# martende/findex

Measured on AMD Instinct MI355X. Metric: rank_queries_per_sec, higher is better.
Workload: dtype u64

## Files before the change

### findex_amd/csrc/fmx_search4.h

```cpp
#pragma once
#include <type_traits>
#include "fmx_device.h"

namespace fmx {

constexpr int kSThreads = 256;

__device__ __forceinline__ uint32_t fetch4(const uint8_t *__restrict__ pat, uint64_t pos) {
  if (pos >= 4) {
    uint32_t d;
    __builtin_memcpy(&d, pat + pos - 4, 4);
    return __builtin_bswap32(d);
  }
  uint32_t r = 0;
  for (uint32_t j = 0; j < (uint32_t)pos; j++) r |= (uint32_t)pat[pos - 1 - j] << (8 * j);
  return r;
}


__device__ __forceinline__ uint32_t pat_chunk(const uint8_t *__restrict__ pat, const uint64_t *__restrict__ own,
                                              uint64_t end, uint32_t len, uint32_t j) {
  const uint32_t have = len > 4u * j ? len - 4u * j : 0u;
  const uint64_t pos = end - 4ull * j;
  const uint32_t back = have >= 4u ? 4u : have;
  const uint8_t *src = have ? pat + (pos - back) : reinterpret_cast<const uint8_t *>(own);
  uint32_t d;
  __builtin_memcpy(&d, src, 4);
  return __builtin_bswap32(d) >> (8u * (4u - (back ? back : 4u)));
}

#ifndef FMX_SEARCH_WAVES
#define FMX_SEARCH_WAVES 6
#endif
#ifdef FMX_SEARCHLOG
static __device__ unsigned long long g_searchlog[1u << 15][4];
#endif
#ifndef FMX_SEARCH_WAVES_G2
#define FMX_SEARCH_WAVES_G2 5
#endif
template <bool WIDE, uint32_t LAYOUT, uint32_t KT, uint32_t JT, uint32_t RW, bool R3T, bool G2 = false, bool KX = false>
__global__ __launch_bounds__(kSThreads) __attribute__((amdgpu_waves_per_eu(G2 ? FMX_SEARCH_WAVES_G2 : FMX_SEARCH_WAVES, 8))) void k_search4(DevIndex ix, const uint4 *__restrict__ ktab, const uint8_t *__restrict__ kdense,
                                                        uint32_t ksigma, const uint4 *__restrict__ kext, const uint4 *__restrict__ kovf,
                                                        const uint4 *__restrict__ jtab, const uint32_t jc,
                                                        const unsigned long long *__restrict__ r3tab, const uint8_t *__restrict__ pat,
                                                        const PatOff po,
                                                        uint64_t *__restrict__ sp_out, uint64_t *__restrict__ ep_out,
                                                        uint32_t k, unsigned long long *__restrict__ counters, const uint64_t pk_cap,
                                                        const uint32_t spin) {
  static_assert(!G2 || LAYOUT == kLayoutOneHot, "pairs of lanes serve the one-hot layout only");
  static_assert(!KX || (KT != 0 && JT == 2u && RW == 0u && LAYOUT == kLayoutOneHot), "level KT + 1 serves the kernels with pairs of row jump entries");
  constexpr int G = G2 ? 2 : Lay<LAYOUT>::G;
  constexpr uint32_t P = 64 / G;
  constexpr uint32_t RG = G2 ? 4u : (uint32_t)G;
  constexpr uint32_t R = LAYOUT == kLayoutBytes ? 2u : 1u;
#ifdef FMX_SEARCHLOG
  const unsigned long long sl_t0 = __builtin_amdgcn_s_memrealtime();
  unsigned long long sl_t1 = 0;
  uint32_t sl_batches = 0;
#endif
  if (threadIdx.x == 0 && blockIdx.x < kCensusBlocks) {
    counters[(size_t)kCounterSlots * kCounterStride + 2u * blockIdx.x] = __builtin_amdgcn_s_memrealtime();
    if (blockIdx.x == 0) counters[(size_t)kCounterSlots * kCounterStride + 2u * kCensusBlocks] = gridDim.x;
  }
  if (spin & 0xFFFFu) {
    const unsigned long long c0 = __builtin_amdgcn_s_memrealtime();
    while (__builtin_amdgcn_s_memrealtime() - c0 < (spin & 0xFFFFu)) __builtin_amdgcn_s_sleep(32);
  }
  __shared__ uint4 s_tab[256];
  __shared__ uint8_t s_dense[KT ? 256 : 4];
  __shared__ uint16_t s_slot[KT ? 256 : 4];
  for (int c = threadIdx.x; c < 256; c += blockDim.x) {
    if (KT) { s_dense[c] = kdense[c]; s_slot[c] = ix.slot[c]; }
    const uint64_t cf = ix.cf[c];
    const uint16_t s = ix.slot[c];
    uint64_t vb = 0;
    if (s < kSlotEof) vb = LAYOUT == kLayoutBytes ? (uint64_t)s + 2 : (uint64_t)(uintptr_t)ix.bv + (uint64_t)s * ix.nblocks * kBlockBytes;
    else if (s == kSlotEof) vb = 1;
    s_tab[c] = make_uint4((uint32_t)cf, (uint32_t)(cf >> 32), (uint32_t)vb, (uint32_t)(vb >> 32));
  }
  __syncthreads();
  const LaneConst lc = lane_const<G2 ? 4 : G>();
  const uint32_t t = G2 ? (threadIdx.x & 1u) : lc.t;
  const uint32_t lane_off = t * 16;
  uint32_t steps = 0, reqs = 0;
  struct Blk { uint4 a, b; };
  auto blk_load = [&](uint64_t vb, uint32_t b1, uint32_t upto) -> Blk {
    const uint64_t at = vb + lane_off + (uint64_t)b1 * kBlockBytes;
    Blk w;
    w.a = load_line16(at);
    w.b = make_uint4(0, 0, 0, 0);
    if constexpr (G2) {
      if (upto >= 192u) w.b = load_line16(at + 32);
    }
    return w;
  };
  auto blk_rank = [&](const Blk &w, uint32_t m1) -> uint64_t {
    if constexpr (G2) return rank_finish_g2<WIDE>(Blk2{w.a, w.b}, m1, t);
    else return rank_finish<WIDE>(w.a, m1, lc);
  };
  auto blk_bit = [&](const Blk &w, uint32_t m1) -> uint32_t {
    if constexpr (G2) return payload_bit_g2(Blk2{w.a, w.b}, m1, t);
    else return payload_bit(w.a, m1, lc);
  };
  constexpr uint32_t RB = 1u;
  auto gbc0 = [&](uint32_t v) -> uint32_t { if constexpr (G2) return pair_bcast<0>(v); else return group_bcast<G, 0>(v); };
  auto gbc1 = [&](uint32_t v) -> uint32_t { if constexpr (G2) return pair_bcast<1>(v); else return group_bcast<G, 1>(v); };
  const uint32_t wave = (blockIdx.x * kSThreads + threadIdx.x) >> 6;
  const uint32_t nwaves = gridDim.x * (kSThreads / 64);
  const uint32_t grp = (threadIdx.x & 63) / G;
  const uint32_t nbatch = (k + P - 1) / P;
  constexpr bool kPool = G2 || RW != 0u;
  const uint32_t tix_area = kPool ? (spin >> 16) & 0xFFu : 0u;
  const bool miss_none = JT != 0u && (spin >> 31) != 0u;
  uint32_t nstatic = nbatch;
  if (tix_area) {
    const uint32_t rounds = nbatch / nwaves, held = (spin >> 24) & 0xFu;
    if (rounds >= held + 2u) nstatic = (rounds - held) * nwaves;
  }
  constexpr bool kStage = LAYOUT != kLayoutBytes;
  constexpr uint32_t kStageBytes = G2 ? 2048 : 1024, kStagePad = 16;
  __shared__ __attribute__((aligned(16))) uint32_t s_pat[kSThreads / 64][2][kStage ? (kStagePad + kStageBytes + 16) / 4 : 4];
  uint32_t par = 0;
  constexpr bool kFold = (JT && RW == 0u) || RW != 0u;
  constexpr uint32_t kParkCap = RW ? 128u : (G2 ? 96u : 64u);
  __shared__ uint64_t s_park_row[kFold ? kSThreads / 64 : 1][kFold ? kParkCap : 1];
  __shared__ uint32_t s_park_pid[kFold ? kSThreads / 64 : 1][kFold ? kParkCap : 1];
  __shared__ uint32_t s_park_it[kFold ? kSThreads / 64 : 1][kFold ? kParkCap : 1];
  uint32_t npark = 0;
  constexpr uint32_t kRowsCap = 64u + P;
  __shared__ uint64_t s_rows_row[RW ? kSThreads / 64 : 1][RW ? kRowsCap : 1];
  __shared__ uint64_t s_rows_end[RW ? kSThreads / 64 : 1][RW ? kRowsCap : 1];
  __shared__ uint32_t s_rows_pid[RW ? kSThreads / 64 : 1][RW ? kRowsCap : 1];
  __shared__ uint32_t s_rows_it[RW ? kSThreads / 64 : 1][RW ? kRowsCap : 1];
  __shared__ uint32_t s_rows_len[RW ? kSThreads / 64 : 1][RW ? kRowsCap : 1];
  uint32_t nrows = 0;
  uint32_t rsteps = 0, rlooks = 0;
  auto emit = [&](uint32_t q, uint64_t a, uint64_t b) {
    if (pk_cap != ~0ull) {
      unsigned long long *pk = reinterpret_cast<unsigned long long *>(sp_out);
      const uint64_t w = b - a;
      if (w >= kPackWide) {
        const unsigned long long slot = atomicAdd(pk + k, 1ull);
        if (slot < pk_cap) { pk[(uint64_t)k + 1 + 2 * slot] = q; pk[(uint64_t)k + 2 + 2 * slot] = b; }
      }
      pk[q] = a | ((w < kPackWide ? w : kPackWide) << 40);
    } else {
      sp_out[q] = a;
      ep_out[q] = b;
    }
  };
  const uint32_t wave_in_wg = (uint32_t)__builtin_amdgcn_readfirstlane((int)(threadIdx.x >> 6));
  const uint32_t lane64 = threadIdx.x & 63u;
  const uint64_t pat_addr = (uint64_t)(uintptr_t)pat;
  auto load_off_raw = [&](uint64_t bt, uint64_t &v0, uint64_t &v1) {
    const uint64_t pid = bt * P + grp;
    const uint64_t *p = po.at(pid < k ? pid : (uint64_t)k - 1);
    v0 = p[0];
    v1 = p[1];
  };
  auto fix_off = [&](uint64_t bt, uint64_t v0, uint64_t v1, uint64_t &e, uint32_t &len) {
    const uint64_t pid = bt * P + grp;
    const uint64_t q = pid < k ? pid : (uint64_t)k - 1;
    const uint64_t b = po.fixed ? q * po.fixed : v0;
    e = po.fixed ? (q + 1) * po.fixed : v1;
    len = pid < k ? (uint32_t)(e - b) : 0u;
  };
  struct Stage { uint4 w; uint4 w2; uint64_t base; bool ok; };
  auto stage_issue = [&](uint64_t e, uint32_t len) {
    const uint64_t b = e - len;
    const uint64_t b0 = ((uint64_t)__builtin_amdgcn_readfirstlane((int)(uint32_t)(b >> 32)) << 32) | (uint32_t)__builtin_amdgcn_readfirstlane((int)(uint32_t)b);
    const uint64_t e1 = ((uint64_t)(uint32_t)__builtin_amdgcn_readlane((int)(uint32_t)(e >> 32), 63) << 32) | (uint32_t)__builtin_amdgcn_readlane((int)(uint32_t)e, 63);
    Stage st;
    const uint64_t al = (pat_addr + b0) & ~15ull;
    const uint64_t span = pat_addr + e1 - al;
    st.ok = kStage && span <= kStageBytes;
    st.base = al - pat_addr;
    st.w = make_uint4(0, 0, 0, 0);
    if (st.ok && 16ull * lane64 < span) st.w = load_line16(al + 16u * lane64);
    st.w2 = make_uint4(0, 0, 0, 0);
    if constexpr (G2) {
      if (st.ok && 1024ull + 16ull * lane64 < span) st.w2 = load_line16(al + 1024u + 16u * lane64);
    }
    return st;
  };
  auto stage_park = [&](const Stage &st, uint32_t area) {
    if (st.ok) *reinterpret_cast<uint4 *>(s_pat[wave_in_wg][area] + (kStagePad + 16u * lane64) / 4) = st.w;
    if constexpr (G2) {
      if (st.ok) *reinterpret_cast<uint4 *>(s_pat[wave_in_wg][area] + (kStagePad + 1024u + 16u * lane64) / 4) = st.w2;
    }
  };
  constexpr uint32_t NT = KT ? KT / 4 : 1;
  struct Tail { uint32_t c[NT]; };
  uint64_t end0, end1, raw2a, raw2b;
  uint32_t len0, len1;
  uint32_t ktl = 0, jtl = 0, r3l = 0;
  {
    uint64_t a0, a1;
    load_off_raw(wave, a0, a1);
    fix_off(wave, a0, a1, end0, len0);
    load_off_raw((uint64_t)wave + nwaves, a0, a1);
    fix_off((uint64_t)wave + nwaves, a0, a1, end1, len1);
  }
  Stage cur = stage_issue(end0, len0);
  stage_park(cur, par);
  Tail tail_ahead;
#pragma unroll
  for (uint32_t i = 0; i < NT; i++) tail_ahead.c[i] = (!kStage && len0 > 4u * i) ? fetch4(pat, end0 - 4ull * i) : 0u;
  auto walk_parked = [&](auto last_tag) {
    constexpr bool kLast = decltype(last_tag)::value;
    while (npark) {
      const uint32_t take = npark < P ? npark : P;
      const bool actw = grp < take;
      const uint32_t slot = npark - take + (actw ? grp : 0u);
      npark -= take;
      const uint32_t wpid = actw ? s_park_pid[wave_in_wg][slot] : 0u;
      uint32_t wit = actw ? s_park_it[wave_in_wg][slot] : 0u;
      uint64_t wsp = actw ? s_park_row[wave_in_wg][slot] : 0ull;
      uint32_t wj = (uint32_t)(wsp >> 56);
      const bool wnone = wj == 0xFFu;
      const bool wkx = KX && actw && wj == 0xFEu;
      wj = (wnone || wkx) ? 0u : wj;
      wsp &= (1ull << 56) - 1;
      if constexpr (R3T && kLast) {
        while (__builtin_amdgcn_ballot_w64(actw && wj >= 3u)) {
          const bool go = actw && wj >= 3u;
          if (go) {
            wsp = r3tab[wsp] & ((1ull << 40) - 1);
            wj -= 3u;
            wit += 3u;
            steps += 3u;
          }
          r3l += (uint32_t)__builtin_popcountll(__builtin_amdgcn_ballot_w64(go && t == 0));
        }
      }
      uint64_t wep = wsp + ((actw && !wnone && !wkx) ? 1u : 0u);
      uint64_t wbegin = 0, wend = 0;
      if (actw) po.get(wpid, wbegin, wend);
      const uint32_t wlen = (uint32_t)(wend - wbegin);
      if constexpr (KX) {
        if (__builtin_amdgcn_ballot_w64(wkx)) {
          uint32_t code = 0;
#pragma unroll
          for (uint32_t j = 0; j < KT; j++) code = code * ksigma + s_dense[wkx ? pat[wend - 1 - j] : 0u];
          const uint4 xe = ktab[wkx ? code : 0u];
          if (wkx) {
            const uint64_t xsp = (((uint64_t)xe.y << 32) | xe.x) & ((1ull << 56) - 1), xep = ((uint64_t)xe.w << 32) | xe.z;
            if (xsp < xep) {
              steps += KT + 1u;
            } else {
              wsp = xsp;
              wep = xep;
              steps += xe.y >> 24;
            }
          }
          ktl += (uint32_t)__builtin_popcountll(__builtin_amdgcn_ballot_w64(wkx && t == 0));
        }
      }
      for (;;) {
        const uint32_t wrem = wlen - wit;
        if (!__builtin_amdgcn_ballot_w64(actw && wsp < wep && wrem != 0u)) break;
        const uint32_t nst = wrem < 8u ? wrem : 8u;
        uint64_t chars = 0;
        if (actw && wsp < wep) {
          if (nst == 8u) {
            uint32_t lo, hi;
            __builtin_memcpy(&lo, pat + (wend - wit - 8), 4);
            __builtin_memcpy(&hi, pat + (wend - wit - 4), 4);
            chars = ((uint64_t)__builtin_bswap32(lo) << 32) | __builtin_bswap32(hi);
          } else {
            for (uint32_t s8 = 0; s8 < nst; s8++) chars |= (uint64_t)pat[wend - wit - 1 - s8] << (8u * s8);
          }
        }
        for (uint32_t s8 = 0; s8 < 8; s8++) {
          const bool stepping = actw && wsp < wep && s8 < nst;
          if (!__builtin_amdgcn_ballot_w64(stepping)) break;
          if (stepping) {
            const uint32_t c = (uint32_t)(chars >> (8u * s8)) & 0xFFu;
            const uint4 en = s_tab[c];
            const uint64_t cfc = ((uint64_t)en.y << 32) | en.x;
            const uint64_t vb = ((uint64_t)en.w << 32) | en.z;
            if (vb > 1) {
              if (LAYOUT == kLayoutBytes) {
                const ByteRankReq q1 = byte_rank_issue(ix, (uint16_t)(vb - 2), wsp, lc);
                wsp = cfc + byte_rank_finish(q1, c, lc);
                wep = wsp + byte_match_bit(q1, c, lc);
              } else {
                uint32_t b1, m1;
                split448(wsp, b1, m1);
                const Blk w1 = blk_load(vb, b1, m1);
                wsp = cfc + blk_rank(w1, m1);
                wep = wsp + blk_bit(w1, m1);
              }
              reqs += R * RB;
            } else {
              const uint64_t r1 = cfc + ((vb == 1 && wsp > ix.eof) ? 1u : 0u);
              wep = cfc + ((vb == 1 && wep > ix.eof) ? 1u : 0u);
              wsp = r1;
            }
            steps++;
          }
        }
        wit += nst;
      }
      if (actw && t == 0) emit(wpid, wsp, wep);
    }
  };
  auto rows_phase = [&](const bool all) {
    if constexpr (RW != 0u) {
      while (nrows >= (all ? 1u : 64u)) {
        const uint32_t take = nrows < 64u ? nrows : 64u;
        const bool on = lane64 < take;
        const uint32_t slot = nrows - take + (on ? lane64 : 0u);
        nrows -= take;
        uint64_t row = on ? s_rows_row[wave_in_wg][slot] : 0ull;
        const uint64_t rend = on ? s_rows_end[wave_in_wg][slot] : 0ull;
        const uint32_t rpid = on ? s_rows_pid[wave_in_wg][slot] : 0u;
        const uint32_t rlen = on ? s_rows_len[wave_in_wg][slot] : 0u;
        uint32_t rit = on ? s_rows_it[wave_in_wg][slot] : 0u;
        bool live = on;
        while (__builtin_amdgcn_ballot_w64(live)) {
          const uint32_t rem = rlen - rit;
          bool fail = false;
          if constexpr (RW == 3u) {
            const bool tm = live && rem >= 3u;
            unsigned long long re = 0;
            uint32_t d = 0;
            if (tm) {
              re = r3tab[row];
              __builtin_memcpy(&d, pat + (rend - rit - 3), 4);
            }
            if (tm && (uint32_t)(re >> 40) == __builtin_bswap32(d << 8)) {
              rlooks++;
              row = re & ((1ull << 40) - 1);
              rit += 3;
              rsteps += 3;
            } else if (live) {
              rlooks += tm ? 1u : 0u;
              if (rem == 0u) emit(rpid, row, row + 1);
              else fail = true;
              live = false;
            }
          } else {
            const bool rm = live && rem != 0u;
            unsigned long long re = 0;
            uint32_t c = 0;
            if (rm) {
              re = r3tab[row];
              c = pat[rend - rit - 1];
            }
            const uint32_t c2 = (uint32_t)(re >> 40) & 0xFFu;
            if (rm && c == c2 && c2 != 0u) {
              rlooks++;
              row = re & ((1ull << 40) - 1);
              rit++;
              rsteps++;
            } else if (live) {
              rlooks += rm ? 1u : 0u;
              if (rem == 0u) emit(rpid, row, row + 1);
              else fail = true;
              live = false;
            }
          }
          const unsigned long long fm = __builtin_amdgcn_ballot_w64(fail);
          if (fm) {
            const uint32_t ps = npark + (uint32_t)__builtin_popcountll(fm & ((1ull << lane64) - 1ull));
            if (fail) { s_park_row[wave_in_wg][ps] = row; s_park_pid[wave_in_wg][ps] = rpid; s_park_it[wave_in_wg][ps] = rit; }
            npark += (uint32_t)__builtin_popcountll(fm);
          }
        }
      }
    }
  };
#ifdef FMX_SEARCHLOG
  sl_t1 = __builtin_amdgcn_s_memrealtime();
#endif
  uint32_t batch = wave;
  Stage nxt_stage;
  {
    auto search_one_batch = [&](auto staged_tag, auto ahead_tag) {
    constexpr bool STAGED = decltype(staged_tag)::value;
    constexpr bool AHEAD = decltype(ahead_tag)::value;
    const uint32_t pid = batch * P + grp;
    const bool act = pid < k;
    const uint64_t *own = po.at(act ? pid : 0u);
    const uint64_t end = end0;
    const uint32_t len = act ? len0 : 0u;
    const uint64_t cur_base = cur.base;
    const uint32_t *const spat = s_pat[wave_in_wg][par];
    auto chunk = [&](uint32_t j) -> uint32_t {
      if constexpr (!STAGED) {
        return pat_chunk(pat, own, end, len, j);
      } else {
        const uint32_t have = len > 4u * j ? len - 4u * j : 0u;
        const uint32_t o = have ? (uint32_t)(end - 4ull * j - cur_base) + (kStagePad - 4u) : 0u;
        const uint32_t lo = spat[o >> 2], hi = spat[(o >> 2) + 1];
        const uint32_t r = __builtin_bswap32(__builtin_amdgcn_alignbyte(hi, lo, o & 3u));
        return have >= 4u ? r : (r & ((1u << (8u * have)) - 1u));
      }
    };
    auto chars4 = [&](uint32_t at) -> uint32_t {
      const uint32_t have = len > at ? len - at : 0u;
      if constexpr (STAGED) {
        const uint32_t o = have ? (uint32_t)(end - at - cur_base) + (kStagePad - 4u) : 0u;
        const uint32_t lo = spat[o >> 2], hi = spat[(o >> 2) + 1];
        const uint32_t r = __builtin_bswap32(__builtin_amdgcn_alignbyte(hi, lo, o & 3u));
        return have >= 4u ? r : (r & ((1u << (8u * have)) - 1u));
      } else {
        uint32_t r = 0;
        if (have >= 4u) {
          uint32_t d;
          __builtin_memcpy(&d, pat + (end - at - 4), 4);
          r = __builtin_bswap32(d);
        } else {
          for (uint32_t j = 0; j < have; j++) r |= (uint32_t)pat[end - at - 1 - j] << (8u * j);
        }
        return r;
      }
    };
    Tail tailq;
#pragma unroll
    for (uint32_t i = 0; i < NT; i++) {
      if constexpr (STAGED) tailq.c[i] = chunk(i);
      else if constexpr (kStage) tailq.c[i] = len > 4u * i ? fetch4(pat, end - 4ull * i) : 0u;
      else tailq.c[i] = act ? tail_ahead.c[i] : 0u;
    }
    uint32_t ch = tailq.c[0];
    uint32_t nx = chunk(KT ? KT / 4 + 1 : 1);
    auto issue_ahead = [&]() {
      if constexpr (AHEAD) {
        nxt_stage = stage_issue(end1, len1);
        if constexpr (!kStage) {
#pragma unroll
          for (uint32_t i = 0; i < NT; i++) tail_ahead.c[i] = len1 > 4u * i ? fetch4(pat, end1 - 4ull * i) : 0u;
        }
        load_off_raw((uint64_t)batch + 2ull * nwaves, raw2a, raw2b);
      }
    };
    if (KT == 0) { issue_ahead(); if constexpr (AHEAD) stage_park(nxt_stage, par ^ 1u); }
    uint64_t sp = 0, ep = ix.n;
    bool kx_parked = false;
    auto special = [&](uint64_t cfc, uint64_t vb, uint64_t x) { return cfc + ((vb == 1 && x > ix.eof) ? 1u : 0u); };
    if (KT == 0) {
      if (len > 0) {
        const uint32_t c = ch & 0xFFu;
        const uint4 e = s_tab[c];
        const uint4 e2 = s_tab[(c + 1) & 0xFFu];
        const uint64_t cfc = ((uint64_t)e.y << 32) | e.x;
        const uint64_t vb = ((uint64_t)e.w << 32) | e.z;
        const uint64_t nxt = c == 255u ? ix.n : (((uint64_t)e2.y << 32) | e2.x);
        sp = vb > 1 ? cfc : special(cfc, vb, 0);
        ep = vb > 1 ? nxt : special(cfc, vb, ix.n);
        steps++;
      }
      ch >>= 8;
    } else {
      uint32_t code = 0;
      bool elig = act && len >= KT;
#pragma unroll
      for (uint32_t j = 0; j < KT; j++) {
        const uint32_t d = s_dense[(tailq.c[j >> 2] >> (8u * (j & 3u))) & 0xFFu];
        elig = elig && d != 0xFFu;
        code = code * ksigma + d;
      }
      bool ex = false;
      uint32_t chk = 0;
      uint32_t zcode = 0;
      if constexpr (KX) {
        chk = chunk(KT / 4);
        bool ez = elig && len > KT;
#pragma unroll
        for (uint32_t j = 1; j <= KT; j++) {
          const uint32_t d = s_dense[((j < KT ? tailq.c[j < KT ? j >> 2 : 0u] : chk) >> (8u * (j & 3u))) & 0xFFu];
          ez = ez && d != 0xFFu;
          zcode = zcode * ksigma + d;
        }
        ex = ez;
      }
      const uint4 *ksrc = ktab + (elig ? code : 0u);
      if constexpr (KX) { if (ex) ksrc = kext + 2ull * zcode + (t & 1u); }
      const uint4 ent = *ksrc;
      issue_ahead();
      if (elig && !ex) {
        sp = (((uint64_t)ent.y << 32) | ent.x) & ((1ull << 56) - 1);
        ep = ((uint64_t)ent.w << 32) | ent.z;
        steps += ent.y >> 24;
      }
      ktl += (uint32_t)__builtin_popcountll(__builtin_amdgcn_ballot_w64(elig && t == 0));
      if constexpr (AHEAD) stage_park(nxt_stage, par ^ 1u);
      if constexpr (KX) {
        if (__builtin_amdgcn_ballot_w64(ex)) {
          const uint32_t half = t & 1u, y = tailq.c[0] & 0xFFu;
          const uint32_t h1 = gbc0(ent.y);
          const bool big = ((h1 >> 8) & 0xFFu) == 0xFFu;
          uint32_t lt = 0, le = 0;
          auto count16 = [&](const uint4 &w, uint32_t from) {
#pragma unroll
            for (uint32_t b = 0; b < 16; b++) {
              const uint32_t x = ((b < 4 ? w.x : b < 8 ? w.y : b < 12 ? w.z : w.w) >> (8u * (b & 3u))) & 0xFFu;
              lt += (b >= from && x < y) ? 1u : 0u;
              le += (b >= from && x <= y) ? 1u : 0u;
            }
          };
          if (ex && !big) count16(ent, half ? 0u : 6u);
          uint32_t cnt = (h1 >> 8) & 0xFFu;
          if (__builtin_amdgcn_ballot_w64(ex && big)) {
            const uint32_t h2 = gbc0(ent.z), h3 = gbc0(ent.w);
            const uint64_t off = (h1 >> 16) | ((uint64_t)(h2 & 0xFFFFFFu) << 16);
            const uint32_t bc = (h2 >> 24) | (h3 << 8);
            if (ex && big) cnt = bc;
            for (uint32_t i = 0;; i++) {
              const bool more = ex && big && 32u * i < bc;
              if (!__builtin_amdgcn_ballot_w64(more)) break;
              uint4 w = make_uint4(~0u, ~0u, ~0u, ~0u);
              if (more && 32u * i + 16u * half < bc) w = kovf[off + 2u * i + half];
              if (more) count16(w, 0u);
              ktl += (uint32_t)__builtin_popcountll(__builtin_amdgcn_ballot_w64(more && t == 0));
            }
          }
          lt = gbc0(lt) + gbc1(lt);
          le = y == 255u ? cnt : gbc0(le) + gbc1(le);
          const uint64_t spz = gbc0(ent.x) | ((uint64_t)(h1 & 0xFFu) << 32);
          if (ex) {
            sp = spz + lt;
            ep = spz + le;
          }
          const bool kxp = ex && sp >= ep;
          const unsigned long long pm = __builtin_amdgcn_ballot_w64(kxp && t == 0);
          if (pm) {
            const uint32_t slot = npark + (uint32_t)__builtin_popcountll(pm & ((1ull << lane64) - 1ull));
            if (kxp && t == 0) { s_park_row[wave_in_wg][slot] = sp | (0xFEull << 56); s_park_pid[wave_in_wg][slot] = pid; s_park_it[wave_in_wg][slot] = KT + 1u; }
            npark += (uint32_t)__builtin_popcountll(pm);
          }
          kx_parked = kxp;
          if (ex && !kxp) steps += KT + 1u;
        }
      }
      constexpr uint32_t kWalk = KX ? KT + 1u : KT;
      if (__builtin_amdgcn_ballot_w64(act && !(KX ? ex : elig))) {
        for (uint32_t j = 0; j < kWalk; j++) {
          const bool stepping = act && (KX ? (!ex && j >= (elig ? KT : 0u)) : !elig) && j < len && sp < ep;
          if (!__builtin_amdgcn_ballot_w64(stepping)) {
            if (KX && j < KT) continue;
            break;
          }
          if (stepping) {
            const uint32_t c = ((j < KT ? tailq.c[j < KT ? j >> 2 : 0u] : chk) >> (8u * (j & 3u))) & 0xFFu;
            const uint4 e = s_tab[c];
            if constexpr (G2) {
              const uint64_t cfc = ((uint64_t)e.y << 32) | e.x, vb = ((uint64_t)e.w << 32) | e.z;
              if (vb > 1) {
                uint32_t b1, b2, m1, m2;
                split448(sp, b1, m1);
                split448(ep, b2, m2);
                const Blk w1 = blk_load(vb, b1, b2 != b1 ? m1 : (m1 > m2 ? m1 : m2));
                Blk w2 = w1;
                if (b2 != b1) { w2 = blk_load(vb, b2, m2); reqs += RB; }
                sp = cfc + blk_rank(w1, m1);
                ep = cfc + blk_rank(w2, m2);
                reqs += RB;
              } else {
                const uint64_t r1 = cfc + ((vb == 1 && sp > ix.eof) ? 1u : 0u);
                ep = cfc + ((vb == 1 && ep > ix.eof) ? 1u : 0u);
                sp = r1;
              }
            } else {
              reqs += backward_step<WIDE, LAYOUT>(ix, c, s_slot[c], ((uint64_t)e.y << 32) | e.x, lc, sp, ep);
            }
            steps++;
          }
        }
      }
      if constexpr (KX) ch = chk >> 8;
      else ch = chunk(KT / 4);
    }
    constexpr uint32_t kIt0 = KX ? KT + 1u : (KT ? KT : 1u);
    uint32_t skip = 0;
    uint32_t cursor_it = kIt0;
    bool deferred = kx_parked;
    for (uint32_t it = kIt0;; it++) {
      bool alive = it < len && sp < ep;
      if constexpr (RW != 0u) {
        const bool hand = alive && (ep - sp) == 1 && (RW == 1u || (len - it) % RW == 0u);
        const unsigned long long hm = __builtin_amdgcn_ballot_w64(hand && t == 0);
        if (hm) {
          const uint32_t slot = nrows + (uint32_t)__builtin_popcountll(hm & ((1ull << lane64) - 1ull));
          if (hand && t == 0) {
            s_rows_row[wave_in_wg][slot] = sp; s_rows_end[wave_in_wg][slot] = end; s_rows_pid[wave_in_wg][slot] = pid;
            s_rows_it[wave_in_wg][slot] = it; s_rows_len[wave_in_wg][slot] = len;
          }
          nrows += (uint32_t)__builtin_popcountll(hm);
        }
        if (hand) {
          deferred = true;
          ep = sp;
          alive = false;
        }
      }
      if (!__builtin_amdgcn_ballot_w64(alive)) break;
      auto cursor_to = [&](uint32_t ni) {
        const uint32_t c0 = chars4(ni), a = ni & 3u;
        ch = a ? (c0 & ((1u << (8u * (4u - a))) - 1u)) : c0;
        nx = chunk((ni >> 2) + 1);
        cursor_it = ni;
      };
      auto chars12 = [&](uint32_t at, bool want, uint32_t &q0, uint32_t &q1, uint32_t &q2) {
        if constexpr (STAGED) {
          const uint32_t o = want ? (uint32_t)(end - at - cur_base) + (kStagePad - 12u) : 0u;
          const uint32_t w0 = o >> 2, sh = o & 3u;
          const uint32_t d0 = spat[w0], d1 = spat[w0 + 1], d2 = spat[w0 + 2], d3 = spat[w0 + 3];
          q0 = __builtin_bswap32(__builtin_amdgcn_alignbyte(d3, d2, sh));
          q1 = __builtin_bswap32(__builtin_amdgcn_alignbyte(d2, d1, sh));
          q2 = __builtin_bswap32(__builtin_amdgcn_alignbyte(d1, d0, sh));
        } else {
          q0 = chars4(at); q1 = chars4(at + 4u); q2 = chars4(at + 8u);
        }
      };
      const uint32_t rem = len - it;
      bool lookedup = false;
      bool park_now = false;
      uint32_t missj = 0;
      uint32_t park_ahead = 0;
      if (JT && !__builtin_amdgcn_ballot_w64(alive && (skip != 0u || (ep - sp) > (uint64_t)RG))) {
        const bool can = alive && rem >= jc;
        if (__builtin_amdgcn_ballot_w64(can)) {
          constexpr bool kPair = JT == 2u && STAGED && (G == 4 || G == 2);
          const uint64_t width = ep - sp;
          const bool single = !__builtin_amdgcn_ballot_w64(can && width != 1u);
          const uint32_t half = (kPair && single) ? (t & 1u) : 0u;
          const bool can2 = kPair && single && can && rem >= 2u * jc;
          uint32_t p0, p1, p2;
          chars12(it + (half && can2 ? jc : 0u), can, p0, p1, p2);
          const uint32_t m2 = jc > 8u ? ((1u << (8u * (jc - 8u))) - 1u) : 0u;
          bool jumped = false, pair_both = false, pair_then_miss = false;
          uint64_t rowj = 0;
          uint32_t nrows = 1;
          if (single) {
            uint4 je = make_uint4(0, 0, 0, 0);
            if (can) je = jtab[(JT == 2u ? 2ull * sp : sp) + (half && can2 ? 1u : 0u)];
            const uint32_t d0 = je.x ^ p0, d1 = je.y ^ p1, d2 = (je.z ^ p2) & m2;
            jumped = can && (d0 | d1 | d2) == 0u;
            missj = d0 ? (uint32_t)__builtin_ctz(d0) >> 3 : (d1 ? 4u + ((uint32_t)__builtin_ctz(d1) >> 3) : 8u + ((uint32_t)__builtin_ctz(d2 | 0x80000000u) >> 3));
            rowj = (uint64_t)(je.z >> 24) | ((uint64_t)je.w << 8);
            if constexpr (kPair) {
              const uint32_t ok = jumped ? 1u : 0u;
              const bool ok1 = gbc0(ok) != 0u, ok2 = can2 && gbc1(ok) != 0u;
              const uint32_t rlo1 = gbc0((uint32_t)rowj), rhi1 = gbc0((uint32_t)(rowj >> 32));
              const uint32_t rlo2 = gbc1((uint32_t)rowj), rhi2 = gbc1((uint32_t)(rowj >> 32));
              const uint32_t mj1 = gbc0(missj), mj2 = gbc1(missj);
              jumped = can && ok1;
              pair_both = ok1 && ok2;
              pair_then_miss = can2 && ok1 && !ok2;
              rowj = pair_both ? (((uint64_t)rhi2 << 32) | rlo2) : (((uint64_t)rhi1 << 32) | rlo1);
              missj = pair_then_miss ? mj2 : mj1;
            }
            jtl += (uint32_t)__builtin_popcountll(__builtin_amdgcn_ballot_w64(can && t == 0));
          } else {
            const uint32_t lane64g = threadIdx.x & 63u, gbase = lane64g - t;
            if constexpr (G2) {
              const bool mn0 = can && (uint64_t)t < width, mn1 = can && (uint64_t)(2u + t) < width;
              uint4 j0 = make_uint4(0, 0, 0, 0), j1 = make_uint4(0, 0, 0, 0);
              if (mn0) j0 = jtab[JT == 2u ? 2ull * (sp + t) : sp + t];
              if (mn1) j1 = jtab[JT == 2u ? 2ull * (sp + 2u + t) : sp + 2u + t];
              const uint32_t d0 = j0.x ^ p0, d1 = j0.y ^ p1, d2 = (j0.z ^ p2) & m2;
              const bool hit0 = mn0 && (d0 | d1 | d2) == 0u;
              const bool hit1 = mn1 && ((j1.x ^ p0) | (j1.y ^ p1) | ((j1.z ^ p2) & m2)) == 0u;
              missj = d0 ? (uint32_t)__builtin_ctz(d0) >> 3 : (d1 ? 4u + ((uint32_t)__builtin_ctz(d1) >> 3) : 8u + ((uint32_t)__builtin_ctz(d2 | 0x80000000u) >> 3));
              const uint32_t hm = ((uint32_t)(__builtin_amdgcn_ballot_w64(hit0) >> gbase) & 3u) | (((uint32_t)(__builtin_amdgcn_ballot_w64(hit1) >> gbase) & 3u) << 2);
              const uint32_t fr = hm ? (uint32_t)__builtin_ctz(hm) : 0u;
              const uint4 js = (fr >> 1) ? j1 : j0;
              const int first = (int)(gbase + (fr & 1u));
              const uint32_t rlo = (uint32_t)__shfl((int)((js.z >> 24) | (js.w << 8)), first, 64), rhi = (uint32_t)__shfl((int)(js.w >> 24), first, 64);
              jumped = can && hm != 0u;
              rowj = ((uint64_t)rhi << 32) | rlo;
              nrows = (uint32_t)__builtin_popcount(hm);
              jtl += (uint32_t)__builtin_popcountll(__builtin_amdgcn_ballot_w64(mn0)) + (uint32_t)__builtin_popcountll(__builtin_amdgcn_ballot_w64(mn1));
            } else {
            const bool mine = can && (uint64_t)t < width;
            uint4 je = make_uint4(0, 0, 0, 0);
            if (mine) je = jtab[JT == 2u ? 2ull * (sp + t) : sp + t];
            const uint32_t d0 = je.x ^ p0, d1 = je.y ^ p1, d2 = (je.z ^ p2) & m2;
            const bool hit = mine && (d0 | d1 | d2) == 0u;
            missj = d0 ? (uint32_t)__builtin_ctz(d0) >> 3 : (d1 ? 4u + ((uint32_t)__builtin_ctz(d1) >> 3) : 8u + ((uint32_t)__builtin_ctz(d2 | 0x80000000u) >> 3));
            const uint32_t hm = (uint32_t)(__builtin_amdgcn_ballot_w64(hit) >> gbase) & ((1u << G) - 1u);
            const int first = (int)(gbase + (hm ? (uint32_t)__builtin_ctz(hm) : 0u));
            const uint32_t rlo = (uint32_t)__shfl((int)((je.z >> 24) | (je.w << 8)), first, 64), rhi = (uint32_t)__shfl((int)(je.w >> 24), first, 64);
            jumped = can && hm != 0u;
            rowj = ((uint64_t)rhi << 32) | rlo;
            nrows = (uint32_t)__builtin_popcount(hm);
            jtl += (uint32_t)__builtin_popcountll(__builtin_amdgcn_ballot_w64(mine));
            }
          }
          if (can) {
            if (!jumped && width == 1u) {
              park_now = true;
              deferred = true;
            }
            const uint32_t took = jumped ? (pair_both ? 2u * jc : jc) : 0u;
            if (pair_then_miss) { park_now = true; deferred = true; park_ahead = jc; }
            ep = (jumped && !pair_then_miss) ? rowj + nrows : ((deferred && !pair_then_miss) ? sp : (pair_then_miss ? rowj : ep));
            sp = jumped ? rowj : sp;
            steps += took;
            skip = pair_then_miss ? 0u : took;
            lookedup = jumped;
          }
        }
      }
      if (JT && R3T) {
        const uint64_t width = ep - sp;
        const bool want3 = alive && skip == 0u && !deferred && !lookedup && width >= 1u && width <= (uint64_t)RG && rem >= 3u &&
                           (rem < jc || it % 3u == 0u);
        if (__builtin_amdgcn_ballot_w64(want3)) {
          const uint32_t three = chars4(it) & 0xFFFFFFu;
          const uint32_t lane64 = threadIdx.x & 63u, base = lane64 - t;
          unsigned long long re = 0;
          uint32_t hm, lo3, hi3;
          bool mine;
          if constexpr (G2) {
            mine = want3 && (uint64_t)t < width;
            const bool mine1 = want3 && (uint64_t)(2u + t) < width;
            unsigned long long re1 = 0;
            if (mine) re = r3tab[sp + t];
            if (mine1) re1 = r3tab[sp + 2u + t];
            const bool h0 = mine && (uint32_t)(re >> 40) == three, h1 = mine1 && (uint32_t)(re1 >> 40) == three;
            hm = ((uint32_t)(__builtin_amdgcn_ballot_w64(h0) >> base) & 3u) | (((uint32_t)(__builtin_amdgcn_ballot_w64(h1) >> base) & 3u) << 2);
            const uint32_t fr = hm ? (uint32_t)__builtin_ctz(hm) : 0u;
            const unsigned long long rs = (fr >> 1) ? re1 : re;
            const int first = (int)(base + (fr & 1u));
            lo3 = (uint32_t)__shfl((int)(uint32_t)rs, first, 64);
            hi3 = (uint32_t)__shfl((int)(uint32_t)(rs >> 32), first, 64);
            r3l += (uint32_t)__builtin_popcountll(__builtin_amdgcn_ballot_w64(mine1));
          } else {
          mine = want3 && (uint64_t)t < width;
          if (mine) re = r3tab[sp + t];
          const bool hit = mine && (uint32_t)(re >> 40) == three;
          hm = (uint32_t)(__builtin_amdgcn_ballot_w64(hit) >> base) & ((1u << G) - 1u);
          const int first = (int)(base + (hm ? (uint32_t)__builtin_ctz(hm) : 0u));
          lo3 = (uint32_t)__shfl((int)(uint32_t)re, first, 64);
          hi3 = (uint32_t)__shfl((int)(uint32_t)(re >> 32), first, 64);
          }
          if (want3) {
            const bool took = hm != 0u;
            if (took) {
              sp = (((uint64_t)hi3 << 32) | lo3) & ((1ull << 40) - 1);
              ep = sp + (uint32_t)__builtin_popcount(hm);
              steps += 3;
              skip = 3u;
              lookedup = true;
            } else if (width == 1u) {
              park_now = true;
              deferred = true;
              ep = sp;
              missj = (uint32_t)__builtin_ctz((((uint32_t)(re >> 40) ^ three) & 0xFFFFFFu) | 0x80000000u) >> 3;
            }
          }
          r3l += (uint32_t)__builtin_popcountll(__builtin_amdgcn_ballot_w64(mine));
        }
      }
      if (JT && __builtin_amdgcn_ballot_w64(park_now)) {
        if constexpr (kFold) {
          if (miss_none && park_now) steps += missj + 1u;
          const unsigned long long pm = __builtin_amdgcn_ballot_w64(park_now && t == 0);
          const uint32_t lane64p = threadIdx.x & 63u;
          const uint32_t slot = npark + (uint32_t)__builtin_popcountll(pm & ((1ull << lane64p) - 1ull));
          if (park_now && t == 0) { s_park_row[wave_in_wg][slot] = miss_none ? (0xFFull << 56) : (sp | ((uint64_t)missj << 56)); s_park_pid[wave_in_wg][slot] = pid; s_park_it[wave_in_wg][slot] = it + park_ahead; }
          npark += (uint32_t)__builtin_popcountll(pm);
        }
      }
      if ((JT || R3T) && !__builtin_amdgcn_ballot_w64(alive && skip == 0u && !deferred)) {
        bool cand = alive && !deferred && skip != 0u;
        uint32_t adv = 0;
#pragma unroll
        for (int bit = (JT == 2u ? 4 : 3); bit >= 0; bit--) {
          const bool z = cand && ((skip >> bit) & 1u) == 0u;
          if (__builtin_amdgcn_ballot_w64(z)) cand = z;
          else adv |= 1u << bit;
        }
        if (!__builtin_amdgcn_ballot_w64(cand)) adv = 1u;
        skip -= skip >= adv ? adv : skip;
        it += adv - 1u;
        continue;
      }
      if constexpr (JT || R3T) {
        if (cursor_it != it) cursor_to(it);
      }
      const bool stepping = alive && skip == 0u && !deferred;
      skip -= skip ? 1u : 0u;
      const bool wide_iv = stepping && (ep - sp) != 1;
      if (!__builtin_amdgcn_ballot_w64(wide_iv)) {
        if (stepping) {
          const uint32_t c = ch & 0xFFu;
          const uint4 e = s_tab[c];
          const uint64_t cfc = ((uint64_t)e.y << 32) | e.x;
          const uint64_t vb = ((uint64_t)e.w << 32) | e.z;
          if (vb > 1) {
            if (LAYOUT == kLayoutBytes) {
              const ByteRankReq q1 = byte_rank_issue(ix, (uint16_t)(vb - 2), sp, lc);
              sp = cfc + byte_rank_finish(q1, c, lc);
              ep = sp + byte_match_bit(q1, c, lc);
            } else {
              uint32_t b1, m1;
              split448(sp, b1, m1);
              const Blk w1 = blk_load(vb, b1, m1);
              sp = cfc + blk_rank(w1, m1);
              ep = sp + blk_bit(w1, m1);
            }
            reqs += R * RB;
          } else {
            const uint64_t r1 = special(cfc, vb, sp);
            ep = special(cfc, vb, ep);
            sp = r1;
          }
          steps++;
        }
      } else if (stepping) {
        const uint32_t c = ch & 0xFFu;
        const uint4 e = s_tab[c];
        const uint64_t cfc = ((uint64_t)e.y << 32) | e.x;
        const uint64_t vb = ((uint64_t)e.w << 32) | e.z;
        if (vb > 1) {
          if (LAYOUT == kLayoutBytes) {
            const ByteRankReq q1 = byte_rank_issue(ix, (uint16_t)(vb - 2), sp, lc);
            ByteRankReq q2 = q1;
            const bool two = (ep >> 7) != (sp >> 7);
            if (two) q2 = byte_rank_issue(ix, (uint16_t)(vb - 2), ep, lc);
            else q2.rem = (uint32_t)ep & 127u;
            sp = cfc + byte_rank_finish(q1, c, lc);
            ep = cfc + byte_rank_finish(q2, c, lc);
            reqs += two ? 2 * R : R;
          } else {
            uint32_t b1, b2, m1, m2;
            split448(sp, b1, m1);
            split448(ep, b2, m2);
            const Blk w1 = blk_load(vb, b1, b2 != b1 ? m1 : (m1 > m2 ? m1 : m2));
            Blk w2 = w1;
            if (b2 != b1) { w2 = blk_load(vb, b2, m2); reqs += RB; }
            sp = cfc + blk_rank(w1, m1);
            ep = cfc + blk_rank(w2, m2);
            reqs += RB;
          }
        } else {
          const uint64_t r1 = special(cfc, vb, sp);
          ep = special(cfc, vb, ep);
          sp = r1;
        }
        steps++;
      }
      ch >>= 8;
      if ((it & 3u) == 3u) {
        ch = nx;
        nx = chunk((it >> 2) + 2);
      }
      cursor_it = it + 1u;
    }
    if (act && t == 0 && !deferred) emit(pid, sp, ep);
    };
    auto one_batch = [&](auto ahead_tag) {
      if constexpr (kStage) {
        if (cur.ok) search_one_batch(std::true_type{}, ahead_tag);
        else search_one_batch(std::false_type{}, ahead_tag);
      } else {
        search_one_batch(std::false_type{}, ahead_tag);
      }
      if constexpr (RW != 0u) {
        if (nrows >= 64u) {
          if (npark > kParkCap - 64u) walk_parked(std::false_type{});
          rows_phase(false);
        }
      } else {
        if (kFold && npark > kParkCap - P) walk_parked(std::false_type{});
      }
    };
    for (; batch < nstatic; batch += nwaves) {
#ifdef FMX_SEARCHLOG
      sl_batches++;
#endif
      one_batch(std::true_type{});
      cur = nxt_stage;
      par ^= 1u;
      end0 = end1; len0 = len1;
      fix_off((uint64_t)batch + 2ull * nwaves, raw2a, raw2b, end1, len1);
    }
    if constexpr (kPool) {
    if (nstatic != nbatch) {
      const uint32_t groups = (nwaves + 31u) >> 5;
      const uint32_t nshards = groups < kTixShards ? groups : kTixShards;
      const uint32_t shard = (wave >> 5) % nshards;
      unsigned long long *tix = counters + (kCounterBytes + kCensusBytes + kCalibScratchBytes) / 8 +
                                ((size_t)(tix_area - 1u) * kTixShards + shard) * kTixStride;
      const uint32_t npool = nbatch - nstatic;
      const uint32_t pool = npool > shard ? (npool - shard + nshards - 1u) / nshards : 0u;
      const uint32_t mine = groups > shard ? (groups - shard + nshards - 1u) / nshards : 0u;
      const uint32_t drawers = mine * 32u - ((groups - 1u) % nshards == shard ? groups * 32u - nwaves : 0u);
      uint32_t drawn = 0;
      if (lane64 == 0) drawn = (uint32_t)atomicAdd(tix, 1ull);
      for (;;) {
        const uint32_t tk = (uint32_t)__builtin_amdgcn_readfirstlane((int)drawn);
        if (tk >= pool) {
          if (tk == pool + drawers - 1u && lane64 == 0) atomicExch(tix, 0ull);
          break;
        }
        if (lane64 == 0) drawn = (uint32_t)atomicAdd(tix, 1ull);
        batch = nstatic + shard + nshards * tk;
#ifdef FMX_SEARCHLOG
        sl_batches++;
#endif
        {
          uint64_t a0, a1;
          load_off_raw(batch, a0, a1);
          fix_off(batch, a0, a1, end0, len0);
        }
        cur = stage_issue(end0, len0);
        stage_park(cur, par);
#pragma unroll
        for (uint32_t i = 0; i < NT; i++) tail_ahead.c[i] = (!kStage && len0 > 4u * i) ? fetch4(pat, end0 - 4ull * i) : 0u;
        one_batch(std::false_type{});
      }
    }
    }
  }
  if constexpr (RW != 0u) {
    if (npark > kParkCap - 64u) walk_parked(std::false_type{});
    rows_phase(true);
  }
#ifdef FMX_SEARCHLOG
  const unsigned long long sl_tw = __builtin_amdgcn_s_memrealtime();
#endif
  if (kFold) walk_parked(std::true_type{});
#ifdef FMX_SEARCHLOG
  const unsigned long long sl_t2 = __builtin_amdgcn_s_memrealtime();
#endif
  counters_add(counters, (t == 0 ? 2ull * steps : 0ull) + 2ull * rsteps, (t == 0 ? steps : 0u) + rsteps, t == 0 ? reqs : 0u);
  if (RW) {
    const unsigned long long rl = wave_sum((unsigned long long)rlooks);
    if ((threadIdx.x & 63u) == 0 && rl) atomicAdd(counters + (size_t)(blockIdx.x % kCounterSlots) * kCounterStride + 11, rl);
  }
#ifdef FMX_SEARCHLOG
  if ((threadIdx.x & 63u) == 0 && wave < (1u << 15)) {
    unsigned long long *e = g_searchlog[wave];
    e[0] = sl_t0; e[1] = ((sl_t1 - sl_t0) & 0xFFFFFFFFull) | ((sl_tw - sl_t0) << 32); e[2] = sl_t2; e[3] = __builtin_amdgcn_s_memrealtime() | ((unsigned long long)sl_batches << 48);
  }
#endif
  if (threadIdx.x == 0 && blockIdx.x < kCensusBlocks)
    counters[(size_t)kCounterSlots * kCounterStride + 2u * blockIdx.x + 1u] = __builtin_amdgcn_s_memrealtime();
  if (KT) {
    const unsigned long long lookups = ktl;
    if ((threadIdx.x & 63u) == 0 && lookups)
      atomicAdd(counters + (size_t)(blockIdx.x % kCounterSlots) * kCounterStride + 9, lookups);
  }
  if (JT) {
    const unsigned long long lookups = jtl;
    if ((threadIdx.x & 63u) == 0 && lookups)
      atomicAdd(counters + (size_t)(blockIdx.x % kCounterSlots) * kCounterStride + 10, lookups);
  }
  if (JT && R3T) {
    const unsigned long long lookups = r3l;
    if ((threadIdx.x & 63u) == 0 && lookups)
      atomicAdd(counters + (size_t)(blockIdx.x % kCounterSlots) * kCounterStride + 11, lookups);
  }
}
struct Search4Args {
  DevIndex ix;
  const uint4 *ktab;
  const uint8_t *kdense;
  uint32_t ksigma;
  const uint4 *kext, *kovf;
  const uint4 *jtab;
  uint32_t jc;
  const unsigned long long *r3tab;
  const uint8_t *pat;
  PatOff po;
  uint64_t *sp_out, *ep_out;
  uint32_t k;
  unsigned long long *counters;
  uint64_t pk_cap;
  uint32_t spin;
};

template <bool WIDE, uint32_t LAYOUT, uint32_t KT, uint32_t JT, uint32_t RW, bool R3T, bool G2, bool KX>
void search4_launch(const Search4Args &a, int grid, hipStream_t st) {
  k_search4<WIDE, LAYOUT, KT, JT, RW, R3T, G2, KX><<<grid, kSThreads, 0, st>>>(a.ix, a.ktab, a.kdense, a.ksigma, a.kext, a.kovf, a.jtab, a.jc, a.r3tab, a.pat, a.po,
                                                                       a.sp_out, a.ep_out, a.k, a.counters, a.pk_cap, a.spin);
}
template <bool WIDE, uint32_t LAYOUT, uint32_t KT, uint32_t JT, uint32_t RW, bool R3T, bool G2, bool KX>
int search4_occupancy() {
  int nb = 0;
  if (hipOccupancyMaxActiveBlocksPerMultiprocessor(&nb, k_search4<WIDE, LAYOUT, KT, JT, RW, R3T, G2, KX>, kSThreads, 0) != hipSuccess) return 0;
  return nb;
}
#ifdef FMX_SEARCHLOG
template <bool WIDE, uint32_t LAYOUT, uint32_t KT, uint32_t JT, uint32_t RW, bool R3T, bool G2, bool KX>
int search4_searchlog(void *out, size_t bytes) {
  return hipMemcpyFromSymbol(out, HIP_SYMBOL(g_searchlog), bytes < sizeof g_searchlog ? bytes : sizeof g_searchlog) == hipSuccess ? 0 : -1;
}
#endif

#define FMX_SEARCH4_ONEHOT_KT(X, W, KT) \
  X(W, kLayoutOneHot, KT, 2, 0, true, true, false) X(W, kLayoutOneHot, KT, 2, 0, true, false, false) \
  X(W, kLayoutOneHot, KT, 1, 0, true, true, false) X(W, kLayoutOneHot, KT, 1, 0, true, false, false) X(W, kLayoutOneHot, KT, 1, 0, false, false, false) \
  X(W, kLayoutOneHot, KT, 0, 3, false, false, false) X(W, kLayoutOneHot, KT, 0, 1, false, false, false) X(W, kLayoutOneHot, KT, 0, 0, false, false, false)
#define FMX_SEARCH4_ONEHOT_KX(X, KT) X(false, kLayoutOneHot, KT, 2, 0, true, true, true) X(false, kLayoutOneHot, KT, 2, 0, true, false, true)
#define FMX_SEARCH4_BYTES_KT(X, KT) \
  X(true, kLayoutBytes, KT, 1, 0, true, false, false) X(true, kLayoutBytes, KT, 1, 0, false, false, false) \
  X(true, kLayoutBytes, KT, 0, 3, false, false, false) X(true, kLayoutBytes, KT, 0, 1, false, false, false) X(true, kLayoutBytes, KT, 0, 0, false, false, false)
#define FMX_SEARCH4_ONEHOT(X, W) \
  FMX_SEARCH4_ONEHOT_KT(X, W, 0) FMX_SEARCH4_ONEHOT_KT(X, W, 4) FMX_SEARCH4_ONEHOT_KT(X, W, 8) FMX_SEARCH4_ONEHOT_KT(X, W, 12)
#define FMX_SEARCH4_ONEHOT_LEVELX(X) FMX_SEARCH4_ONEHOT_KX(X, 4) FMX_SEARCH4_ONEHOT_KX(X, 8) FMX_SEARCH4_ONEHOT_KX(X, 12)
#define FMX_SEARCH4_BYTES(X) FMX_SEARCH4_BYTES_KT(X, 0) FMX_SEARCH4_BYTES_KT(X, 4) FMX_SEARCH4_BYTES_KT(X, 8) FMX_SEARCH4_BYTES_KT(X, 12)
#define FMX_SEARCH4_LIST(X) FMX_SEARCH4_ONEHOT(X, false) FMX_SEARCH4_ONEHOT(X, true) FMX_SEARCH4_BYTES(X) FMX_SEARCH4_ONEHOT_LEVELX(X)

#ifdef FMX_SEARCHLOG
#define FMX_SEARCH4_SEARCHLOG_(D, W, L, KT, JT, RW, R3T, G2, KX) D int search4_searchlog<W, L, KT, JT, RW, R3T, G2, KX>(void *, size_t);
#else
#define FMX_SEARCH4_SEARCHLOG_(D, W, L, KT, JT, RW, R3T, G2, KX)
#endif
#define FMX_SEARCH4_WRAPPERS_(D, W, L, KT, JT, RW, R3T, G2, KX)                                    \
  D void search4_launch<W, L, KT, JT, RW, R3T, G2, KX>(const Search4Args &, int, hipStream_t);     \
  D int search4_occupancy<W, L, KT, JT, RW, R3T, G2, KX>();                                        \
  FMX_SEARCH4_SEARCHLOG_(D, W, L, KT, JT, RW, R3T, G2, KX)
#define FMX_SEARCH4_EXTERN(W, L, KT, JT, RW, R3T, G2, KX) FMX_SEARCH4_WRAPPERS_(extern template, W, L, KT, JT, RW, R3T, G2, KX)
#define FMX_SEARCH4_INSTANTIATE(W, L, KT, JT, RW, R3T, G2, KX) FMX_SEARCH4_WRAPPERS_(template, W, L, KT, JT, RW, R3T, G2, KX)
FMX_SEARCH4_LIST(FMX_SEARCH4_EXTERN)

}
```

Before: 553,000.

## Prefetch next batch's k-mer table entry one batch ahead in staged KX kernel

```diff
diff --git a/findex_amd/csrc/fmx_search4.h b/findex_amd/csrc/fmx_search4.h
--- a/findex_amd/csrc/fmx_search4.h
+++ b/findex_amd/csrc/fmx_search4.h
@@ -38,8 +38,14 @@
 #ifndef FMX_SEARCH_WAVES_G2
 #define FMX_SEARCH_WAVES_G2 5
 #endif
+#ifndef FMX_SEARCH_AHEAD
+#define FMX_SEARCH_AHEAD 1
+#endif
+#ifndef FMX_SEARCH_WAVES_AHEAD
+#define FMX_SEARCH_WAVES_AHEAD FMX_SEARCH_WAVES_G2
+#endif
 template <bool WIDE, uint32_t LAYOUT, uint32_t KT, uint32_t JT, uint32_t RW, bool R3T, bool G2 = false, bool KX = false>
-__global__ __launch_bounds__(kSThreads) __attribute__((amdgpu_waves_per_eu(G2 ? FMX_SEARCH_WAVES_G2 : FMX_SEARCH_WAVES, 8))) void k_search4(DevIndex ix, const uint4 *__restrict__ ktab, const uint8_t *__restrict__ kdense,
+__global__ __launch_bounds__(kSThreads) __attribute__((amdgpu_waves_per_eu(G2 ? (KX && KT == 4u && FMX_SEARCH_AHEAD ? FMX_SEARCH_WAVES_AHEAD : FMX_SEARCH_WAVES_G2) : FMX_SEARCH_WAVES, 8))) void k_search4(DevIndex ix, const uint4 *__restrict__ ktab, const uint8_t *__restrict__ kdense,
                                                         uint32_t ksigma, const uint4 *__restrict__ kext, const uint4 *__restrict__ kovf,
                                                         const uint4 *__restrict__ jtab, const uint32_t jc,
                                                         const unsigned long long *__restrict__ r3tab, const uint8_t *__restrict__ pat,
@@ -203,6 +209,43 @@
   }
   Stage cur = stage_issue(end0, len0);
   stage_park(cur, par);
+  constexpr bool kAhead = FMX_SEARCH_AHEAD != 0 && kStage && KX && G2 && KT == 4u;
+  uint4 ent_ahead;
+  auto entry_issue = [&](uint32_t area, uint64_t e, uint32_t len, uint64_t base) {
+    if constexpr (kAhead) {
+      const uint32_t *const sa = s_pat[wave_in_wg][area];
+      uint32_t c[NT + 1];
+#pragma unroll
+      for (uint32_t j = 0; j <= NT; j++) {
+        const uint32_t have = len > 4u * j ? len - 4u * j : 0u;
+        const uint32_t o = have ? (uint32_t)(e - 4ull * j - base) + (kStagePad - 4u) : 0u;
+        const uint32_t lo = sa[o >> 2], hi = sa[(o >> 2) + 1];
+        const uint32_t r = __builtin_bswap32(__builtin_amdgcn_alignbyte(hi, lo, o & 3u));
+        c[j] = have >= 4u ? r : (r & ((1u << (8u * have)) - 1u));
+      }
+      uint32_t code = 0, zcode = 0;
+      bool elig = len >= KT;
+#pragma unroll
+      for (uint32_t j = 0; j < KT; j++) {
+        const uint32_t d = s_dense[(c[j >> 2] >> (8u * (j & 3u))) & 0xFFu];
+        elig = elig && d != 0xFFu;
+        code = code * ksigma + d;
+      }
+      bool ex = elig && len > KT;
+#pragma unroll
+      for (uint32_t j = 1; j <= KT; j++) {
+        const uint32_t d = s_dense[(c[j >> 2] >> (8u * (j & 3u))) & 0xFFu];
+        ex = ex && d != 0xFFu;
+        zcode = zcode * ksigma + d;
+      }
+      const uint4 *ksrc = ktab + (elig ? code : 0u);
+      if (ex) ksrc = kext + 2ull * zcode + (t & 1u);
+      ent_ahead = *ksrc;
+    }
+  };
+  if constexpr (kAhead) {
+    if (cur.ok && wave < nstatic) entry_issue(par, end0, len0, cur.base);
+  }
   Tail tail_ahead;
 #pragma unroll
   for (uint32_t i = 0; i < NT; i++) tail_ahead.c[i] = (!kStage && len0 > 4u * i) ? fetch4(pat, end0 - 4ull * i) : 0u;
@@ -380,6 +423,23 @@
     auto search_one_batch = [&](auto staged_tag, auto ahead_tag) {
     constexpr bool STAGED = decltype(staged_tag)::value;
     constexpr bool AHEAD = decltype(ahead_tag)::value;
+    constexpr bool kFromAhead = kAhead && STAGED && AHEAD;
+    auto next_entry = [&]() {
+      if constexpr (kAhead) {
+      if constexpr (kFromAhead) load_off_raw((uint64_t)batch + 2ull * nwaves, raw2a, raw2b);
+      stage_park(nxt_stage, par ^ 1u);
+      if (nxt_stage.ok && (uint64_t)batch + nwaves < nstatic) entry_issue(par ^ 1u, end1, len1, nxt_stage.base);
+      }
+    };
+    auto entry_taken = [&]() -> uint4 {
+      uint4 e = make_uint4(0, 0, 0, 0);
+      if constexpr (kAhead) {
+        e = ent_ahead;
+        asm volatile("" : "+v"(e.x), "+v"(e.y), "+v"(e.z), "+v"(e.w));
+      }
+      return e;
+    };
+    [[maybe_unused]] bool ahead_due = kFromAhead;
     const uint32_t pid = batch * P + grp;
     const bool act = pid < k;
     const uint64_t *own = po.at(act ? pid : 0u);
@@ -433,7 +493,7 @@
 #pragma unroll
           for (uint32_t i = 0; i < NT; i++) tail_ahead.c[i] = len1 > 4u * i ? fetch4(pat, end1 - 4ull * i) : 0u;
         }
-        load_off_raw((uint64_t)batch + 2ull * nwaves, raw2a, raw2b);
+        if constexpr (!kFromAhead) load_off_raw((uint64_t)batch + 2ull * nwaves, raw2a, raw2b);
       }
     };
     if (KT == 0) { issue_ahead(); if constexpr (AHEAD) stage_park(nxt_stage, par ^ 1u); }
@@ -478,7 +538,7 @@
       }
       const uint4 *ksrc = ktab + (elig ? code : 0u);
       if constexpr (KX) { if (ex) ksrc = kext + 2ull * zcode + (t & 1u); }
-      const uint4 ent = *ksrc;
+      const uint4 ent = kFromAhead ? entry_taken() : *ksrc;
       issue_ahead();
       if (elig && !ex) {
         sp = (((uint64_t)ent.y << 32) | ent.x) & ((1ull << 56) - 1);
@@ -486,7 +546,8 @@
         steps += ent.y >> 24;
       }
       ktl += (uint32_t)__builtin_popcountll(__builtin_amdgcn_ballot_w64(elig && t == 0));
-      if constexpr (AHEAD) stage_park(nxt_stage, par ^ 1u);
+      if constexpr (AHEAD && !kAhead) stage_park(nxt_stage, par ^ 1u);
+      if constexpr (kAhead && AHEAD && !kFromAhead) next_entry();
       if constexpr (KX) {
         if (__builtin_amdgcn_ballot_w64(ex)) {
           const uint32_t half = t & 1u, y = tailq.c[0] & 0xFFu;
@@ -594,6 +655,12 @@
           deferred = true;
           ep = sp;
           alive = false;
+        }
+      }
+      if constexpr (kFromAhead) {
+        if (ahead_due && it != kIt0) {
+          next_entry();
+          ahead_due = false;
         }
       }
       if (!__builtin_amdgcn_ballot_w64(alive)) break;
@@ -852,6 +919,9 @@
       }
       cursor_it = it + 1u;
     }
+    if constexpr (kFromAhead) {
+      if (ahead_due) next_entry();
+    }
     if (act && t == 0 && !deferred) emit(pid, sp, ep);
     };
     auto one_batch = [&](auto ahead_tag) {
@@ -878,6 +948,9 @@
       cur = nxt_stage;
       par ^= 1u;
       end0 = end1; len0 = len1;
+      if constexpr (kAhead) {
+        asm volatile("" : "+v"(raw2a), "+v"(raw2b));
+      }
       fix_off((uint64_t)batch + 2ull * nwaves, raw2a, raw2b, end1, len1);
     }
     if constexpr (kPool) {
```

Measured after the change: 483,100. -12.6%, worse.
